# url-kaist/UV-SLAM

Measured on AMD Instinct MI355X. Metric: sliding-window solves/sec (10 KF, 150 pts, 40 lines, 3 VP), higher is better.
Workload: dtype f64; 1 GPU; W10-P150-L40-V3 x 256 independent windows per GPU (BASELINE configs[2]); single window (configs[1]) in single_window, the 20k-point window (configs[3]) in large_window (both with --full); windows_per_gpu=256, frames=11, points=150, lines=40, vp_tagged_lines=30, prior=True, parallelism=replicas x1

## Files before the change

uv-slam_amd/csrc/uvs_solve_kernel.h:

```cpp
#pragma once
#include <hip/hip_runtime.h>
#include <initializer_list>
#include <utility>
#include "../../include/uvs_solver.h"
#include "uvs_layout.h"
#include "uvs_factors.h"

namespace uvsdev {

#ifndef UVS_UNIT
#define UVS_UNIT unit
#endif

#ifndef UVS_X_PLAIN_TID
static __device__ __forceinline__ int lane_tid() { int t = threadIdx.x; asm volatile("" : "+v"(t)); return t; }
#else
static __device__ __forceinline__ int lane_tid() { return threadIdx.x; }
#endif
static constexpr int NT = UVS_NT;
static constexpr int NW = NT / 64;
static constexpr bool ROLES = NT > 256;
static constexpr int ET = ROLES ? 256 : NT;
static constexpr int EW = ET / 64;
static constexpr int GT0 = NT - UVS_GT;
// ... 219 lines not shown
            for (int k = 0; k < 9; ++k) x0[k] = x0g[k];
        }
        const double* xb = (kind == UVS_BLOCK_POSE) ? x + 7 * frame : (kind == UVS_BLOCK_SPEEDBIAS) ? x + 77 + 9 * frame : (kind == UVS_BLOCK_TD) ? x + 183 : x + 176;
        double* dx = c.sh + L_PDX + idx;
        if (size != 7) { for (int k = 0; k < size; ++k) dx[k] = xb[k] - x0[k]; }
        else {
            dx[0] = xb[0] - x0[0]; dx[1] = xb[1] - x0[1]; dx[2] = xb[2] - x0[2];
            double qi[4], e[4]; quat_inv(x0 + 3, qi); quat_mul(qi, xb + 3, e);
            const double sg = (e[3] >= 0.0) ? 2.0 : -2.0;
            dx[3] = sg * e[0]; dx[4] = sg * e[1]; dx[5] = sg * e[2];
        }
    }
}
UVS_DEV double prior_quad(const Ctx& c, int dst = L_PR) {
    DevWinK& h = *c.hdr;
    const int n = h.prior_n, tid = lane_tid();
    double cost = 0.0;
    if (n <= 0) return cost;
    const double* H0 = c.ws + h.w_prior_h0;
    const int parts = (NT / n) < 4 ? (NT / n) : 4;
    const int part = tid / n, row = tid - part * n;
    const double g0v = tid < n ? c.ws[h.w_prior_h0 + UVS_PH_G0(n) + tid] : 0.0, c0v = tid == 0 ? c.ws[h.w_prior_h0 + UVS_PH_C0(n)] : 0.0;
    if (part < parts) {
        const int kb = (n * part) / parts, ke = (n * (part + 1)) / parts;
        double p8[8] = {0, 0, 0, 0, 0, 0, 0, 0};
        for (int k = kb; k < ke; k += PR_UN) {
            double jv[PR_UN];
#pragma unroll
            for (int u = 0; u < PR_UN; ++u) jv[u] = H0[(k + u < ke ? k + u : kb) * n + row];
#pragma unroll
            for (int u = 0; u < PR_UN; ++u) if (k + u < ke) p8[u & 7] += jv[u] * c.sh[L_PDX + k + u];
        }
        c.sh[L_S + 128 * part + row] = ((p8[0] + p8[1]) + (p8[2] + p8[3])) + ((p8[4] + p8[5]) + (p8[6] + p8[7]));
    }
    __syncthreads();
    if (tid < n) {
        double y = c.sh[L_S + tid];
        for (int p = 1; p < parts; ++p) y += c.sh[L_S + 128 * p + tid];
        c.sh[dst + tid] = y;
        cost = c.sh[L_PDX + tid] * (g0v + 0.5 * y);
        if (tid == 0) cost += c0v;
    }
    return cost;
}
UVS_DEV double prior_cost_share(const Ctx& c, int src) {
    DevWinK& h = *c.hdr;
    const int n = h.prior_n, tid = lane_tid();
    double cost = 0.0;
    if (tid < n) {
        cost = c.sh[L_PDX + tid] * (c.ws[h.w_prior_h0 + UVS_PH_G0(n) + tid] + 0.5 * c.sh[src + tid]);
        if (tid == 0) cost += c.ws[h.w_prior_h0 + UVS_PH_C0(n)];
    }
    return cost;
}
UVS_DEV double prior_residual_rows(const Ctx& c) {
    DevWinK& h = *c.hdr;
    const int n = h.prior_n, tid = lane_tid();
    double cost = 0.0;
    if (tid < n) {
        const double* Jr = c.bd + h.d_prior + (size_t)tid * n;
        double s = c.bd[h.d_prior + n * n + tid];
        for (int k = 0; k < n; ++k) s += Jr[k] * c.sh[L_PDX + k];
        c.sh[L_PR + tid] = s;
        cost = 0.5 * s * s;
    }
    return cost;
}

UVS_DEV void cost_imu_raw(const Ctx& c, const double* x, int lane0) {
    DevWinK& h = *c.hdr;
    const int b = lane_tid() - lane0;
    double* rs = c.sh + L_S + 1024;
    if (b >= 0 && b < h.n_imu) {
        const int fi = c.bi[h.i_imu + 2 * b], skip = c.bi[h.i_imu + 2 * b + 1];
        if (!skip) {
            const double* blk = c.bd + h.d_imu + (size_t)b * UVS_IMU_STRIDE;
            double r[15];
            imu_raw(blk, blk + UVS_IMU_JAC, c.o.G, x + 7 * fi, x + 77 + 9 * fi, x + 7 * (fi + 1), x + 77 + 9 * (fi + 1), r, nullptr);
#pragma unroll
            for (int i = 0; i < 15; ++i) rs[16 * b + i] = r[i];
        }
    }
}
template <int PB = CP_PB, int LB = CP_LB>
UVS_DEV double cost_pass(const Ctx& c, const double* x, const double* invd, const double* line, int po0, int po1, int lo0, int lo1, bool with_imu) {
    DevWinK& h = *c.hdr;
    const int tid = lane_tid();
    const double* RF = c.sh + L_RF; const double* ric = c.sh + L_EX; const double* tic = c.sh + L_EX + 9;
    const double* ltrig = line_trig_of(c, line);
    double cost = 0.0;
    long long tq_ = clock64();
#define UVS_CQ(slot) if (c.o.debug == 1 && tid == 0) { const long long t_ = clock64(); c.sh[L_WPROF + slot] += (double)(t_ - tq_); tq_ = t_; }
    const int imu_lane0 = ROLES ? NT - 64 : 0;
#ifndef UVS_X_NO_IMU_WAVE
    if (ROLES && with_imu) cost_imu_raw(c, x, imu_lane0);
#endif
    for (int o0 = po0 + tid; o0 < po1; o0 += PB * NT) {
        int lm[PB], fi[PB], fj[PB]; bool in[PB];
        double pi[PB][3], pj[PB][3], vij[PB][4], idp[PB];
#pragma unroll
        for (int u = 0; u < PB; ++u) {
            const int o = o0 + u * NT; in[u] = o < po1;
            const int oo = in[u] ? o : o0;
            lm[u] = c.bi[h.i_pt_lm + oo]; fi[u] = c.bi[h.i_pt_fi + oo]; fj[u] = c.bi[h.i_pt_fj + oo];
            load_point_obs(c, oo, x[183], pi[u], pj[u], vij[u]);
        }
#pragma unroll
        for (int u = 0; u < PB; ++u) idp[u] = invd[lm[u]];
#pragma unroll
        for (int u = 0; u < PB; ++u) {
            if (!in[u]) continue;
            double r[2];
            point_eval<false, false>(x + 7 * fi[u], RF + 9 * fi[u], pose_of(x, fj[u]), RF + 9 * fj[u], ric, tic, idp[u], pi[u], pj[u], c.o.sqrt_info, r, nullptr, nullptr, nullptr, nullptr);
            double sc; cost += 0.5 * cauchy(c.o.loss_pt, r[0] * r[0] + r[1] * r[1], &sc);
        }
    }
    for (int o0 = lo0 + UVS_COST_LINE_LANE; o0 < lo1; o0 += LB * NT) {
        int lm[LB], fj[LB], hv[LB]; bool in[LB];
        double ms[LB][9], lp[LB][4] = {}, tg[LB][8];
        const int st = h.ln_stride;
#pragma unroll
        for (int u = 0; u < LB; ++u) {
            const int o = o0 + u * NT; in[u] = o < lo1;
            const int oo = in[u] ? o : o0;
            lm[u] = c.bi[h.i_ln_lm + oo]; fj[u] = c.bi[h.i_ln_fj + oo]; hv[u] = c.bi[h.i_ln_vp + oo];
            const double* m = c.bd + h.d_lnmeas + oo;
#pragma unroll
            for (int q = 0; q < 9; ++q) ms[u][q] = m[q * st];
        }
#pragma unroll
        for (int u = 0; u < LB; ++u) {
            if (ltrig) {
#pragma unroll
                for (int q = 0; q < 8; ++q) tg[u][q] = ltrig[8 * lm[u] + q];
            } else {
#pragma unroll
                for (int q = 0; q < 4; ++q) lp[u][q] = line[4 * lm[u] + q];
            }
        }
#pragma unroll
        for (int u = 0; u < LB; ++u) {
            if (!in[u]) continue;
            const double sp[3] = {ms[u][0], ms[u][1], ms[u][2]}, ep[3] = {ms[u][3], ms[u][4], ms[u][5]}, vp[3] = {ms[u][6], ms[u][7], ms[u][8]};
            LineGeom g;
            line_geom<false>(x + 7 * fj[u], x + 7 * fj[u] + 3, RF + 9 * fj[u], ric, tic, lp[u], g, ltrig ? tg[u] : nullptr);
            double r[2], sc;
            line_residual<false>(g, sp, ep, c.o.line_factor, r, nullptr, nullptr);
            cost += 0.5 * cauchy(c.o.loss_ln, r[0] * r[0] + r[1] * r[1], &sc);
            if (hv[u]) { double rv; vp_residual<false>(g, vp, c.o.vp_factor, &rv, nullptr, nullptr); cost += 0.5 * cauchy(c.o.loss_vp, rv * rv, &sc); }
        }
    }
    UVS_CQ(2)
    if (with_imu) {
        double* rs = c.sh + L_S + 1024;
#ifndef UVS_X_NO_IMU_WAVE
        if (!ROLES)
#endif
        cost_imu_raw(c, x, 0);
        __syncthreads();
        const int b = tid >> 4, i = tid & 15;
        if (b < h.n_imu && i < 15 && !c.bi[h.i_imu + 2 * b + 1]) {
            const double* W = c.ws + h.w_imu_w + (size_t)b * UVS_IMU_WS + i * 15;
            double wv[15];
#pragma unroll
            for (int k = 0; k < 15; ++k) wv[k] = (k >= i) ? W[k] : 0.0;
            double sacc = 0.0;
#pragma unroll
            for (int k = 0; k < 15; ++k) sacc += wv[k] * rs[16 * b + k];
            cost += 0.5 * sacc * sacc;
        }
    }
    UVS_CQ(3)
    return cost;
}

typedef double d4_t __attribute__((ext_vector_type(4)));

UVS_DEV double* sblk(double* sh, int i, int j) { return sh + L_S + (((i * (i + 1)) >> 1) + j) * UVS_BLK_SZ; }

UVS_DEV double rcp_newton(double x) {
    double y = __builtin_amdgcn_rcp(x);
    double e = fma(-x, y, 1.0); y = fma(y, e, y);
    e = fma(-x, y, 1.0); y = fma(y, e, y);
    return y;
}

struct MiniCtx { double* sh; struct { int debug; } o; };
template <bool TR = false>
UVS_DEV void chol_update_item(double* sh, int i, int cc, int j0, int j1, int lane, d4_t& acc) {
    const int li = lane & 15, lk = lane >> 4;
    const bool rhs = (i == UVS_NF);
    const double* Bj = sblk(sh, cc, j0) + li * UVS_BLK_LD + lk;
    const double* Ai = rhs ? sh + L_DLT + 16 * j0 + lk : sblk(sh, i, j0) + li * UVS_BLK_LD + lk;
    const int astep = rhs ? 16 : UVS_BLK_SZ;
    if (j0 >= j1) return;
    double a0[4], b0[4], a1[4], b1[4];
#define UVS_CH_LOAD(AV, BV) { _Pragma("unroll") for (int q = 0; q < 4; ++q) { AV[q] = Ai[4 * q]; BV[q] = Bj[4 * q]; } Bj += UVS_BLK_SZ; Ai += astep; }
#define UVS_CH_MFMA(AV, BV) { _Pragma("unroll") for (int q = 0; q < 4; ++q) acc = TR ? __builtin_amdgcn_mfma_f64_16x16x4f64(BV[q], AV[q], acc, 0, 0, 1) : __builtin_amdgcn_mfma_f64_16x16x4f64(AV[q], BV[q], acc, 0, 0, 1); }
    UVS_CH_LOAD(a0, b0)
    for (int j = j0;;) {
        if (j + 1 < j1) UVS_CH_LOAD(a1, b1)
        UVS_CH_MFMA(a0, b0)
        if (++j >= j1) break;
        if (j + 1 < j1) UVS_CH_LOAD(a0, b0)
        UVS_CH_MFMA(a1, b1)
        if (++j >= j1) break;
    }
#undef UVS_CH_LOAD
#undef UVS_CH_MFMA
}
UVS_DEV d4_t chol_load_item(double* sh, int i, int cc, int lane) {
    const int li = lane & 15, lk = lane >> 4;
    d4_t acc;
    if (i == UVS_NF) { const double bv0 = sh[L_DLT + 16 * cc + li]; acc[0] = (lk == 0) ? bv0 : 0.0; acc[1] = 0.0; acc[2] = 0.0; acc[3] = 0.0; }
    else if (i == cc) {
        const double* Dk = sblk(sh, cc, cc);
#pragma unroll
        for (int q = 0; q < 4; ++q) { const int r = lk + 4 * q; const int hi_ = r >= li ? r : li, lo_ = r >= li ? li : r; acc[q] = Dk[hi_ * UVS_BLK_LD + lo_]; }
    } else {
        const double* Cb = sblk(sh, i, cc) + lk * UVS_BLK_LD + li;
#pragma unroll
        for (int q = 0; q < 4; ++q) acc[q] = Cb[4 * q * UVS_BLK_LD];
    }
    return acc;
}
UVS_DEV d4_t chol_load_item_t(double* sh, int i, int cc, int lane) {
    const int li = lane & 15, lk = lane >> 4;
    d4_t acc;
    if (i != UVS_NF) {
        const double* Ai = sblk(sh, i, cc) + li * UVS_BLK_LD + lk;
#pragma unroll
        for (int q = 0; q < 4; ++q) acc[q] = Ai[4 * q];
    } else {
#pragma unroll
        for (int q = 0; q < 4; ++q) { const double yv = sh[L_DLT + 16 * cc + 4 * q + lk]; acc[q] = (li == 0) ? yv : 0.0; }
    }
    return acc;
}
UVS_DEV void chol_store_item(double* sh, int i, int cc, int lane, const d4_t& acc) {
    const int li = lane & 15, lk = lane >> 4;
    if (i == UVS_NF) { if (lk == 0) sh[L_DLT + 16 * cc + li] = acc[0]; }
    else if (i == cc) {
// ... 637 lines not shown
#pragma unroll
                for (int r = 0; r < GR; ++r) { o.p0[r] = pa[r]; o.p1[r] = pa[p1off + r]; }
#pragma unroll
                for (int k = 0; k < 3; ++k) { o.q0[k] = lds2(pb + 2 * k); o.q1[k] = lds2(pb + 6 + 2 * k); }
                o.rc = lds2(S0 + lo + ((w[0] & UVS_PT_ENTRY_A) ? UVS_PT_RC2 - UVS_PT_A : rcoff));
            },
            [&](int, Ops& o) {
#pragma unroll
                for (int r = 0; r < GR; ++r) {
                    if (dirv) { row_fma(A.v + 6 * r, o.p0[r], o.q0); row_fma(A.v + 6 * r, o.p1[r], o.q1); }
                    if (tdcol) A.v[6 * r] += o.p0[r] * o.q0[0].x + o.p1[r] * o.q0[0].y;
                    if (diag) { A.g[r] += o.p0[r] * o.rc.x + o.p1[r] * o.rc.y; A.hd[r] += o.p0[r] * o.p0[r] + o.p1[r] * o.p1[r]; }
                }
            });
    }
}

template <bool DELTA = false>
UVS_DEV void gather_lines(int grp, const int* lists, const double* S0, GAcc& A, int goff = 0, int eoff = 0) {
    const int g = (lane_tid() - GT0) / UVS_GLANES, r0 = GR * (lane_tid() % UVS_GLANES);
    const bool on = grp >= 0;
    const bool diag = on && ((grp >> 8) & 1);
    const int* ent = lists + LIST_HDR;
    {
        struct Ops { double ea[4][GR]; d2_t y[4][3]; double gg[DELTA ? GR : 1]; };
        const int e0 = on ? lists[g] : 0, e1 = on ? lists[g + 1] : 0;
        gather_walk<1, Ops>(ent, e0, e1,
            [&](int, const int* w, Ops& o) {
                const int lo = w[0] & 0x7fff;
                const double* pa = S0 + lo + r0;
                const double* pb = S0 + ((unsigned)w[0] >> 16);
#pragma unroll
                for (int q = 0; q < 4; ++q) {
#pragma unroll
                    for (int r = 0; r < GR; ++r) o.ea[q][r] = pa[6 * q + r];
                    o.y[q][0] = lds2(pb + 6 * q); o.y[q][1] = lds2(pb + 6 * q + 2); o.y[q][2] = lds2(pb + 6 * q + 4);
                }
                if (DELTA) {
                    const double* pg = S0 + goff + 6 * ((lo - eoff) / UVS_LN_EY) + r0;
#pragma unroll
                    for (int r = 0; r < GR; ++r) o.gg[r] = pg[r];
                }
            },
            [&](int, Ops& o) {
#pragma unroll
                for (int q = 0; q < 4; ++q)
#pragma unroll
                    for (int r = 0; r < GR; ++r) row_fma(A.v + 6 * r, -o.ea[q][r], o.y[q]);
                if (DELTA) {
#pragma unroll
                    for (int r = 0; r < GR; ++r) A.g[r] -= diag ? o.gg[r] : 0.0;
                }
            });
    }
    if (DELTA) return;
    {
        struct Ops { double p[3][GR]; d2_t q[3][3], rc01; double rc2; };
        const int e0 = on ? lists[UVS_NGRP + 1 + g] : 0, e1 = on ? lists[UVS_NGRP + 2 + g] : 0;
        gather_walk<1, Ops>(ent, e0, e1,
            [&](int, const int* w, Ops& o) {
                const double* R = S0 + w[0];
#pragma unroll
                for (int k = 0; k < 3; ++k) {
#pragma unroll
                    for (int r = 0; r < GR; ++r) o.p[k][r] = R[UVS_LN_JP + 6 * k + r0 + r];
                    o.q[k][0] = lds2(R + UVS_LN_JP + 6 * k); o.q[k][1] = lds2(R + UVS_LN_JP + 6 * k + 2); o.q[k][2] = lds2(R + UVS_LN_JP + 6 * k + 4);
                }
                o.rc01 = lds2(R); o.rc2 = R[UVS_LN_RV];
            },
            [&](int, Ops& o) {
#pragma unroll
                for (int r = 0; r < GR; ++r) {
#pragma unroll
                    for (int k = 0; k < 3; ++k) { row_fma(A.v + 6 * r, o.p[k][r], o.q[k]); A.hd[r] += o.p[k][r] * o.p[k][r]; }
                    A.g[r] += o.p[0][r] * o.rc01.x + o.p[1][r] * o.rc01.y + o.p[2][r] * o.rc2;
                }
            });
    }
}

static constexpr int IMU_JLD = 48;
static constexpr int IMU_WOFF = 16 * IMU_JLD;
static constexpr int IMU_BLK = IMU_WOFF + UVS_BLK_SZ;
#ifndef UVS_IMU_SLOT_SWAP
#define UVS_IMU_SLOT_SWAP 1
#endif
static constexpr int IMU_SLOTS = (UVS_NF - 1 + NW - 1) / NW;
UVS_DEV int imu_block_of(int wv, int s) {
    if (NW == 8 && UVS_IMU_SLOT_SWAP) return s == 0 ? wv : (wv == 0 ? 9 : wv == 1 ? 8 : UVS_NF);
    return wv + s * NW;
}
struct ImuN { d4_t n00[IMU_SLOTS], n10[IMU_SLOTS], n11[IMU_SLOTS]; int fi[IMU_SLOTS]; bool act[IMU_SLOTS]; };

UVS_DEV double lin_prep(const Ctx& c, const double* x, int mode = 0) {
    UVS_PROF(c, P_MISC);
    const int tid = lane_tid(), n = c.hdr->prior_n;
    if (mode == 0) {
        stage_rotations(c, x);
        prior_dx(c, x);
        __syncthreads();
        return prior_quad(c);
    }
    if (mode == 2) { stage_rotations(c, x); prior_dx(c, x); __syncthreads(); }
    else if (tid < n) c.sh[L_PR + tid] = c.sh[L_PRC + tid];
    __syncthreads();
    return prior_cost_share(c, L_PR);
}
UVS_DEV void lin_imu_stage(const Ctx& c, const double* x) {
    DevWinK& h = *c.hdr;
    double* sh = c.sh;
    const int tid = lane_tid(), lane = tid & 63, wv = tid >> 6;
    __syncthreads();
    UVS_PROF(c, P_GATHER);
    double* IM = sh + L_S;
    constexpr int WPL = ((UVS_NF - 1) * 225 + ET - 1) / ET;
    double wreg[WPL];
#pragma unroll
    for (int q = 0; q < WPL; ++q) {
        const int t = tid + q * ET, tc = t < h.n_imu * 225 ? t : 0, b = tc / 225, e = tc - 225 * b;
        wreg[q] = c.ws[h.w_imu_w + (size_t)b * UVS_IMU_WS + e];
    }
    for (int t = tid; t < h.n_imu * IMU_BLK; t += ET) IM[t] = 0.0;
    UVS_TLOG(c, 40);
    __syncthreads();
    UVS_TLOG(c, 41);
    if (lane < h.n_imu && wv < 4 && !c.bi[h.i_imu + 2 * lane + 1]) {
        const int fi = c.bi[h.i_imu + 2 * lane];
        const double* blk = c.bd + h.d_imu + (size_t)lane * UVS_IMU_STRIDE;
        double* T = IM + IMU_BLK * lane;
        const double* pi_ = x + 7 * fi; const double* si_ = x + 77 + 9 * fi; const double* pj_ = x + 7 * (fi + 1); const double* sj_ = x + 77 + 9 * (fi + 1);
        double r[15];
        if (EW < 4) { imu_raw<IMU_JLD, 1, false>(blk, blk + UVS_IMU_JAC, c.o.G, pi_, si_, pj_, sj_, r, T); for (int i = 0; i < 15; ++i) T[i * IMU_JLD + 31] = r[i]; }
        else if (wv == 0) { imu_raw<IMU_JLD, 1, false, 1>(blk, blk + UVS_IMU_JAC, c.o.G, pi_, si_, pj_, sj_, r, T); for (int i = 0; i < 15; ++i) T[i * IMU_JLD + 31] = r[i]; }
        else if (wv == 1) imu_raw<IMU_JLD, 1, false, 2>(blk, blk + UVS_IMU_JAC, c.o.G, pi_, si_, pj_, sj_, r, T);
        else if (wv == 2) imu_raw<IMU_JLD, 1, false, 4>(blk, blk + UVS_IMU_JAC, c.o.G, pi_, si_, pj_, sj_, r, T);
        else imu_raw<IMU_JLD, 1, false, 8>(blk, blk + UVS_IMU_JAC, c.o.G, pi_, si_, pj_, sj_, r, T);
    }
#pragma unroll
    for (int q = 0; q < WPL; ++q) {
        const int t = tid + q * ET;
        if (t < h.n_imu * 225) { const int b = t / 225, e = t - 225 * b, i = e / 15, k = e - 15 * i; IM[IMU_BLK * b + IMU_WOFF + i * UVS_BLK_LD + k] = wreg[q]; }
    }
    UVS_TLOG(c, 42);
    __syncthreads();
    UVS_TLOG(c, 43);
}
UVS_DEV double lin_imu_tiles(const Ctx& c, ImuN& N) {
    DevWinK& h = *c.hdr;
    double* sh = c.sh;
    const int tid = lane_tid(), lane = tid & 63, wv = UVS_KWAVE(tid), li = lane & 15, lk = lane >> 4;
    double cost = 0.0;
    double* IM = sh + L_S;
    IntK* itab = (IntK*)c.bi + h.i_imu;
    bool act[IMU_SLOTS];
#pragma unroll
    for (int s = 0; s < IMU_SLOTS; ++s) {
        const int b = imu_block_of(wv, s);
        act[s] = b < h.n_imu && !itab[2 * (b < h.n_imu ? b : 0) + 1];
        N.act[s] = act[s]; N.fi[s] = itab[2 * (b < h.n_imu ? b : 0)];
        if (act[s]) {
            double* Jb = IM + IMU_BLK * b; const double* Wb = Jb + IMU_WOFF;
            d4_t t0 = {0.0, 0.0, 0.0, 0.0}, t1 = t0;
            double wa[4], j0[4], j1[4];
#pragma unroll
            for (int q = 0; q < 4; ++q) { wa[q] = Wb[li * UVS_BLK_LD + 4 * q + lk]; j0[q] = Jb[(4 * q + lk) * IMU_JLD + li]; j1[q] = Jb[(4 * q + lk) * IMU_JLD + 16 + li]; }
#pragma unroll
            for (int q = 0; q < 4; ++q) { t0 = __builtin_amdgcn_mfma_f64_16x16x4f64(wa[q], j0[q], t0, 0, 0, 0); t1 = __builtin_amdgcn_mfma_f64_16x16x4f64(wa[q], j1[q], t1, 0, 0, 0); }
#pragma unroll
            for (int q = 0; q < 4; ++q) { Jb[(lk + 4 * q) * IMU_JLD + li] = t0[q]; Jb[(lk + 4 * q) * IMU_JLD + 16 + li] = t1[q]; }
        }
    }
    wave_sync();
#pragma unroll
    for (int s = 0; s < IMU_SLOTS; ++s) {
        const int b = imu_block_of(wv, s);
        d4_t n00 = {0.0, 0.0, 0.0, 0.0}, n10 = n00, n11 = n00;
        if (act[s]) {
            const double* Jb = IM + IMU_BLK * b;
            double j0[4], j1[4];
#pragma unroll
            for (int q = 0; q < 4; ++q) { j0[q] = Jb[(4 * q + lk) * IMU_JLD + li]; j1[q] = Jb[(4 * q + lk) * IMU_JLD + 16 + li]; }
#pragma unroll
            for (int q = 0; q < 4; ++q) {
                n00 = __builtin_amdgcn_mfma_f64_16x16x4f64(j0[q], j0[q], n00, 0, 0, 0);
                n10 = __builtin_amdgcn_mfma_f64_16x16x4f64(j1[q], j0[q], n10, 0, 0, 0);
                n11 = __builtin_amdgcn_mfma_f64_16x16x4f64(j1[q], j1[q], n11, 0, 0, 0);
            }
            if (lane == 63) cost += 0.5 * n11[3];
        }
        N.n00[s] = n00; N.n10[s] = n10; N.n11[s] = n11;
    }
    UVS_PROF(c, P_AS_IMU);
    return cost;
}
UVS_DEV double lin_imu(const Ctx& c, const double* x, ImuN& N) { lin_imu_stage(c, x); return lin_imu_tiles(c, N); }
UVS_DEV double lin_frames(const Ctx& c, const double* x, ImuN& N) { const double pc = lin_prep(c, x); return pc + lin_imu(c, x, N); }

UVS_DEV void spd4_inverse(const double* H, const double* gl, double* X, double* hg) {
    double L[10];
    double i0, i1, i2, i3;
    rsqrt_pair(H[0], &L[0], &i0);
    L[1] = H[1] * i0; rsqrt_pair(H[2] - L[1] * L[1], &L[2], &i1);
    L[3] = H[3] * i0; L[4] = (H[4] - L[3] * L[1]) * i1; rsqrt_pair(H[5] - L[3] * L[3] - L[4] * L[4], &L[5], &i2);
    L[6] = H[6] * i0; L[7] = (H[7] - L[6] * L[1]) * i1; L[8] = (H[8] - L[6] * L[3] - L[7] * L[4]) * i2;
    rsqrt_pair(H[9] - L[6] * L[6] - L[7] * L[7] - L[8] * L[8], &L[9], &i3);
// ... 873 lines not shown
    }
    if (mode != 2) asm_prior(c);
    __syncthreads();
    UVS_PROF(c, P_AS_ADD);
    if (mode == 1) return;
    asm_finish(c, x, first, radius, cost, gmax_lm, mode);
    UVS_PROF(c, P_ASSEMBLE);
}

static constexpr int ROLE_PARTS_OFF = (UVS_NF - 1) * IMU_BLK;
static_assert(ROLE_PARTS_OFF + (8 * GR + 1) * UVS_GT <= UVS_S_DOUBLES, "IMU staging + part sums exceed the S region");
UVS_DEV void role_barriers(int n) { for (int i = 0; i < n; ++i) __syncthreads(); }
UVS_DEV void gacc_store(const Ctx& c, const GAcc& A) {
    double* W = c.ws + c.hdr->w_gacc + (lane_tid() - GT0);
#pragma unroll
    for (int q = 0; q < 6 * GR; ++q) __builtin_nontemporal_store(A.v[q], W + q * UVS_GT);
#pragma unroll
    for (int q = 0; q < GR; ++q) { __builtin_nontemporal_store(A.g[q], W + (6 * GR + q) * UVS_GT); __builtin_nontemporal_store(A.hd[q], W + (7 * GR + q) * UVS_GT); }
}
UVS_DEV void gacc_load(const Ctx& c, GAcc& A) {
    const double* W = c.ws + c.hdr->w_gacc + (lane_tid() - GT0);
#pragma unroll
    for (int q = 0; q < 6 * GR; ++q) A.v[q] = W[q * UVS_GT];
#pragma unroll
    for (int q = 0; q < GR; ++q) { A.g[q] = W[(6 * GR + q) * UVS_GT]; A.hd[q] = W[(7 * GR + q) * UVS_GT]; }
}
UVS_DEV void linearize_roles(const Ctx& c, const double* x, const double* invd, const double* line, bool first, double radius, int prep_mode, bool redamp) {
    DevWinK& h = *c.hdr;
    const bool ev = role_eval();
    { const double pc = lin_prep(c, x, redamp ? 2 : prep_mode); if (!redamp) lacc_set(c.sh, pc, 0.0); }
    double ic = 0.0;
    UVS_TLOG(c, 20);
    PriorAdd pa;
    ImuN N;
    if (ev) {
        ChunkDesc d = chunk_desc(c, 0);
        for (int ch = 0; ch < h.n_chunks; ++ch) {
            if (redamp) redamp_prep(c, d, radius);
            else {
                chunk_eval(c, d, x, invd, line, first, radius);
            }
            if (ch + 1 < h.n_chunks) {
                d = chunk_desc(c, ch + 1);
#ifdef UVS_CHUNK_TOUCH
                if (!redamp) chunk_touch(c, d, invd, line);
#endif
            }
        }
        UVS_TLOG(c, 21);
        lin_imu_stage(c, x);
#ifndef UVS_X_NO_PRIOR_AHEAD
        asm_prior_load(c, pa);
#endif
        ic = lin_imu_tiles(c, N);
        UVS_TLOG(c, 22);
        __syncthreads();
        asm_zero(c);
        __syncthreads();
        UVS_TLOG(c, 23);
        __syncthreads();
        UVS_TLOG(c, 24);
        asm_imu(c, N);
        UVS_TLOG(c, 25);
    } else {
        const int grp = gather_group(c);
        GAcc A;
        if (redamp) gacc_load(c, A); else gacc_zero(A);
        ChunkDesc d = chunk_desc(c, 0);
        for (int ch = 0; ch < h.n_chunks; ++ch) {
            if (redamp) { role_barriers(redamp_barriers(d)); redamp_gather(c, d, grp, A); }
            else {
                __syncthreads();
                if (LISTS_BY_GATHERERS) copy_lists_gatherers(c, d);
                AnchorPre ap; ap.b0 = 0; ap.b1 = 0; ap.sc = 1.0;
                if (ANCHOR_BY_GATHERERS && d.type == 0) pt_anchor_pre(c, d, first, ap);
                __syncthreads();
                if (ANCHOR_BY_GATHERERS && d.type == 0) pt_anchor_pass(c, d, first, radius, ap);
                role_barriers(chunk_eval_barriers(d) - 2);
                chunk_gather(c, d, grp, A);
            }
            if (ch + 1 < h.n_chunks) d = chunk_desc(c, ch + 1);
        }
        __syncthreads();
        if (h.redamp_ok && c.o.redamp) gacc_store(c, A);
        GAcc& T = A;
        gacc_gather_parts(T, grp, c.sh + L_S + ROLE_PARTS_OFF);
#ifndef UVS_X_NO_PRIOR_AHEAD
        asm_prior_load(c, pa);
#endif
        ic = lin_imu_tiles(c, N);
        __syncthreads();
        asm_zero(c);
        __syncthreads();
        asm_part0(c, grp, T);
        __syncthreads();
        asm_imu(c, N);
    }
#ifndef UVS_X_NO_PRIOR_AHEAD
    asm_prior_add(c, pa);
#else
    asm_prior(c);
#endif
    __syncthreads();
    UVS_TLOG(c, 26);
    asm_finish(c, x, first && !redamp, radius, lacc_cost(c.sh) + ic, lacc_gmax(c.sh), 0);
    UVS_TLOG(c, 27);
}

UVS_DEV void linearize(const Ctx& c, const double* x, const double* invd, const double* line, bool first, double radius, int prep_mode, GAcc& A) {
    if (ROLES) { linearize_roles(c, x, invd, line, first, radius, prep_mode, false); return; }
    DevWinK& h = *c.hdr;
    const int grp = gather_group(c);
    gacc_zero(A);
    { const double pc = lin_prep(c, x, prep_mode); lacc_set(c.sh, pc, 0.0); }
    {
        ChunkDesc d = chunk_desc(c, 0);
        for (int ch = 0; ch < h.n_chunks; ++ch) {
            chunk_eval(c, d, x, invd, line, first, radius);
            chunk_gather(c, d, grp, A);
            if (ch + 1 < h.n_chunks) d = chunk_desc(c, ch + 1);
        }
    }
    ImuN N;
    const double ic = lin_imu(c, x, N);
    lin_assemble(c, x, first, radius, grp, A, N, lacc_cost(c.sh) + ic, lacc_gmax(c.sh));
}

UVS_DEV void relinearize_damping(const Ctx& c, const double* x, double radius, GAcc& A) {
    if (ROLES) { linearize_roles(c, x, nullptr, nullptr, false, radius, 2, true); return; }
    DevWinK& h = *c.hdr;
    const int grp = gather_group(c);
    (void)lin_prep(c, x, 2);
    {
        ChunkDesc d = chunk_desc(c, 0);
        for (int ch = 0; ch < h.n_chunks; ++ch) {
            redamp_prep(c, d, radius);
            redamp_gather(c, d, grp, A);
            if (ch + 1 < h.n_chunks) d = chunk_desc(c, ch + 1);
        }
    }
    ImuN N;
    const double ic = lin_imu(c, x, N);
    lin_assemble(c, x, false, radius, grp, A, N, lacc_cost(c.sh) + ic, lacc_gmax(c.sh));
}

#ifndef UVS_BS_FRAME_LANE0
#define UVS_BS_FRAME_LANE0 192
#endif
template <int LNBT = BS_LNB, int PSB = 4, bool STREAM = false>
UVS_DEV void backsub_candidate(const Ctx& c, const double* invd, const double* line, double* invd_c, double* line_c,
                                  int pk0, int pk1, int lk0, int lk1, bool with_frames, double* sums_out, double* lstep = nullptr) {
    DevWinK& h = *c.hdr;
    double* sh = c.sh;
    const int tid = lane_tid();
    const double* d = sh + L_DLT;
    double gd = 0.0, dd2 = 0.0, step2 = 0.0, xc2 = 0.0;
    const bool td_on = UVS_KPIN(h.td_on) != 0;
    const bool ex_on = UVS_KPIN(h.ex_on) != 0, relo_on = h.relo_on != 0;
    double* ltrig_c = const_cast<double*>(line_trig_of(c, line_c));
    const bool relo2 = h.relo2 != 0;
    const int i_pt_fi = UVS_KPIN(h.i_pt_fi), i_pt_fj = UVS_KPIN(h.i_pt_fj), i_ln_fj = UVS_KPIN(h.i_ln_fj), pt_xslots = UVS_KPIN(h.pt_xslots);
    if (relo2) relo2_backsub(c);
    else if (relo_on) {
        if (tid < 6) sh[L_DLT + 16 * UVS_RELO_FRAME + tid] = d[UVS_EX_INDEX(tid)];
        __syncthreads();
    }
    if (with_frames && tid < UVS_RD && ((tid & 15) < 15 || (td_on && tid == UVS_TD_INDEX) || ((ex_on | relo_on) && tid < 96))) { gd += sh[L_G + tid] * d[tid]; dd2 += sh[L_DD + tid] * d[tid] * d[tid]; }
// ... 356 lines not shown
    const long long t_wall0 = wall_clock64();
    while (true) {
        if (it >= o.max_it && !first) { term = UVS_TERM_NO_CONVERGENCE; break; }
        if (o.max_ticks > 0 && !first) {
            __syncthreads();
            if (tid == 0) sh[L_CTRL + C_TIMEUP] = (wall_clock64() - t_wall0 >= o.max_ticks) ? 1.0 : 0.0;
            __syncthreads();
            if (sh[L_CTRL + C_TIMEUP] != 0.0) { term = UVS_TERM_MAX_TIME; break; }
        }
        if (need_lin) {
#ifndef UVS_X_NO_REDAMP
            if (prep_mode == 2 && !first && h.redamp_ok && o.redamp) relinearize_damping(c, sh + L_X, radius, gacc);
            else
#endif
            linearize(c, sh + L_X, invd[cur], line[cur], first, radius, prep_mode, gacc);
            need_lin = false;
            const double lc = sh[L_CTRL + C_COST];
            gmax = sh[L_CTRL + C_GMAX];
            if (first) {
                const double xn2 = ambient_sqnorm(c, sh + L_X, invd[0], line[0]);
                x_norm = sqrt(xn2); cost = lc; first = false;
                if (tid == 0) { rep->initial_cost = cost; rep->cost[0] = cost; rep->radius[0] = radius; rep->gradient_max_norm[0] = gmax; rep->accepted[0] = 1; }
                if (!isfinite(cost)) { term = UVS_TERM_NUMERIC_FAILURE; status = UVS_ERR_NUMERIC; break; }
            } else if (pending > 0) {
                cost = lc;
                if (tid == 0) { rep->cost[pending] = cost; rep->gradient_max_norm[pending] = gmax; }
            }
            pending = 0;
        }
        if (it >= o.max_it) { term = UVS_TERM_NO_CONVERGENCE; break; }
        if (gmax <= o.gtol) { term = UVS_TERM_GRADIENT_TOL; break; }
        if (radius <= o.rmin) { term = UVS_TERM_MIN_RADIUS; break; }
        ++it;
        const int ti = it < UVS_MAX_ITER ? it : UVS_MAX_ITER;
        if (tid < UVS_RD) sh[L_DLT + tid] = -sh[L_G + tid];
        if (o.debug && it == 1 && dbg.S) {
            __syncthreads();
            for (int t = tid; t < UVS_RD * UVS_RD; t += NT) { const int i = t / UVS_RD, j = t - i * UVS_RD; dbg.S[t] = (j <= i) ? sh[L_S + sidx(i, j)] : 0.0; }
            if (tid < UVS_RD) { dbg.g[tid] = sh[L_G + tid]; dbg.hd[tid] = sh[L_HD + tid]; dbg.dd[tid] = sh[L_DD + tid]; }
        }
        UVS_PROF(c, P_MISC);
        UVS_TLOG(c, 30);
        chol_factor(c);
        UVS_PROF(c, P_CHOL);
        UVS_TLOG(c, 31);
        chol_solve(c);
        UVS_PROF(c, P_TRSV);
        UVS_TLOG(c, 32);
        bool ok = sh[L_CTRL + C_CHOLOK] != 0.0;
        backsub_candidate(c, invd[cur], line[cur], invd[cur ^ 1], line[cur ^ 1], 0, h.n_points, 0, h.n_lines, true, nullptr,
                          DSTEP ? ds.steps + (size_t)(it - 1) * ds.stride + UVS_DSTEP_FR : nullptr);
        UVS_PROF(c, P_BACKSUB);
        UVS_TLOG(c, 33);
        const double mcc = sh[L_CTRL + C_MCC], step2 = sh[L_CTRL + C_STEP2], xc2 = sh[L_CTRL + C_XC2];
        if (DSTEP) {
            if (tid < UVS_DSTEP_FR) ds.steps[(size_t)(it - 1) * ds.stride + tid] = sh[L_DLT + tid];
            if (tid == 0) { double* sc = ds.scal + (size_t)(it - 1) * UVS_DEBUG_SCAL_LEN; sc[0] = cost; sc[1] = gmax; sc[2] = ok ? 1.0 : 0.0; sc[3] = mcc; sc[4] = step2; }
            if (it >= ds.n) break;
            radius = ds.radii[it]; need_lin = true; prep_mode = 2;
            __syncthreads();
            continue;
        }
        if (o.debug && it == 1 && dbg.S) {
            if (tid < UVS_RD) dbg.step[tid] = sh[L_DLT + tid];
            if (tid == 0) { dbg.scal[0] = cost; dbg.scal[1] = gmax; dbg.scal[2] = ok ? 1.0 : 0.0; dbg.scal[3] = mcc; dbg.scal[4] = step2; }
        }
        if (!isfinite(mcc) || !isfinite(step2)) ok = false;
        if (tid == 0) rep->model_cost_change[ti] = mcc;
        if (!ok || !(mcc > 0.0)) {
            ++invalid;
            radius = radius / decr; decr *= 2.0; need_lin = true; prep_mode = 2;
            if (tid == 0) { rep->accepted[ti] = -1; rep->cost[ti] = cost; rep->candidate_cost[ti] = cost; rep->radius[ti] = radius; rep->gradient_max_norm[ti] = gmax; }
            if (invalid >= o.max_invalid) { term = UVS_TERM_INVALID_STEPS; break; }
            continue;
        }
        invalid = 0;
        __syncthreads();
        long long tc_ = clock64();
        stage_rotations(c, sh + L_XC);
        prior_dx(c, sh + L_XC);
        __syncthreads();
        if (o.debug == 1 && tid == 0) { const long long t_ = clock64(); sh[L_WPROF + 0] += (double)(t_ - tc_); tc_ = t_; }
        UVS_TLOG(c, 34);
        double cc_ = prior_quad(c, L_PRC);
        UVS_TLOG(c, 35);
        if (o.debug == 1 && tid == 0) { const long long t_ = clock64(); sh[L_WPROF + 1] += (double)(t_ - tc_); tc_ = t_; }
        cc_ += cost_pass(c, sh + L_XC, invd[cur ^ 1], line[cur ^ 1], 0, h.n_pt_obs, 0, h.n_ln_obs, true);
        UVS_TLOG(c, 36);
        double s4[4] = {cc_, 0, 0, 0}, mx = 0.0;
        block_reduce(sh, s4, &mx);
        UVS_TLOG(c, 37);
        UVS_PROF(c, P_COST);
        double cand = s4[0];
        if (!isfinite(cand)) cand = 1.7976931348623157e308;
        const double step_norm = sqrt(step2);
        const double rel = (cost - cand) / mcc;
        const bool successful = rel > o.min_rel;
        if (tid == 0) { rep->candidate_cost[ti] = cand; rep->step_norm[ti] = step_norm; rep->relative_decrease[ti] = rel; rep->cost[ti] = cost; rep->radius[ti] = radius; rep->gradient_max_norm[ti] = gmax; }
        bool stop = false;
        if (step_norm <= o.ptol * (x_norm + o.ptol)) { term = UVS_TERM_PARAMETER_TOL; stop = true; }
        else if (fabs(cost - cand) <= o.ftol * cost) { term = UVS_TERM_FUNCTION_TOL; stop = true; }
        if (stop && !(o.keep_cand && successful)) break;
        if (successful) {
            __syncthreads();
            if (tid < UVS_XDIM) sh[L_X + tid] = sh[L_XC + tid];
            cur ^= 1; ++nsucc;
            x_norm = sqrt(xc2);
            { const double t3 = 2.0 * rel - 1.0; radius = radius / fmax(1.0 / 3.0, 1.0 - t3 * t3 * t3); }
            radius = fmin(o.rmax, radius);
            decr = 2.0;
            cost = cand;
            need_lin = true; pending = ti; prep_mode = 1;
            if (tid == 0) { rep->accepted[ti] = 1; rep->cost[ti] = cost; rep->radius[ti] = radius; }
            if (stop) break;
        } else {
            radius = radius / decr; decr *= 2.0; need_lin = true; prep_mode = 2;
            if (tid == 0) { rep->accepted[ti] = 0; rep->radius[ti] = radius; }
        }
    }
    __syncthreads();
    UVS_PROF(c, P_MISC);
    if (o.debug && dbg.scal && tid < P_LAST) dbg.scal[8 + tid] = sh[L_PROF + tid];
    if (o.debug && dbg.scal && tid < 8) dbg.scal[24 + tid] = sh[L_WPROF + tid];
    if (tid < UVS_XDIM) c.ws[h.w_out + tid] = sh[L_X + tid];
    for (int k = tid; k < h.n_points; k += NT) c.ws[h.w_out + UVS_XDIM + k] = invd[cur][k];
    for (int k = tid; k < 4 * h.n_lines; k += NT) c.ws[h.w_out + UVS_XDIM + h.n_points + k] = line[cur][k];
    if (h.out_host) {
        double* od = (double*)h.out_host;
        if (tid < UVS_XDIM) od[tid] = sh[L_X + tid];
        for (int k = tid; k < h.n_points; k += NT) od[UVS_XDIM + k] = invd[cur][k];
        for (int k = tid; k < 4 * h.n_lines; k += NT) od[UVS_XDIM + h.n_points + k] = line[cur][k];
    }
    if (tid == 0) {
        rep->status = status; rep->termination = term; rep->num_iterations = it; rep->num_successful = nsucc; rep->final_cost = cost;
        ((DevWin*)blob)->cur_sel = cur;
    }
}
#ifdef UVS_EMIT_K_SOLVE
__global__ __launch_bounds__(NT) void k_solve(char* blobs, const long long* blob_off, double* ws_all, const long long* ws_off,
                                              KOpts o, uvs_report* reports, DebugOut dbg) {
    extern __shared__ __attribute__((aligned(16))) double sh[];
    k_solve_body<false>(blobs, blob_off, ws_all, ws_off, o, reports, dbg, DebugStep{}, sh);
}
#endif
#ifdef UVS_EMIT_K_SOLVE_DSTEP
__global__ __launch_bounds__(NT) void k_solve_dstep(char* blobs, const long long* blob_off, double* ws_all, const long long* ws_off,
                                                    KOpts o, uvs_report* reports, DebugStep ds) {
    extern __shared__ __attribute__((aligned(16))) double sh[];
    DebugOut dbg; dbg.S = nullptr; dbg.g = nullptr; dbg.hd = nullptr; dbg.dd = nullptr; dbg.step = nullptr; dbg.scal = nullptr;
    k_solve_body<true>(blobs, blob_off, ws_all, ws_off, o, reports, dbg, ds, sh);
}
#endif

static int unit_init(const unsigned char* fa, const unsigned char* fb, int n, std::initializer_list<const void*> kernels) {
    if (n != UVS_NBLK) return UVS_ERR_INVALID_ARG;
    if (hipMemcpyToSymbol(HIP_SYMBOL(c_blk_fa), fa, n) != hipSuccess || hipMemcpyToSymbol(HIP_SYMBOL(c_blk_fb), fb, n) != hipSuccess) return UVS_ERR_HIP;
    for (const void* fn : kernels) if (hipFuncSetAttribute(fn, hipFuncAttributeMaxDynamicSharedMemorySize, (int)LDS_BYTES) != hipSuccess) return UVS_ERR_HIP;
    return UVS_OK;
}
}
```

Before: 192,300 solves/s.

## Fold prior cost into per-thread partials and widen IMU tile zeroing

New measurement: 192,700 solves/s, median of 3. Within noise of the previous version (+0.2%).

```diff
diff --git a/uv-slam_amd/csrc/uvs_solve_kernel.h b/uv-slam_amd/csrc/uvs_solve_kernel.h
--- a/uv-slam_amd/csrc/uvs_solve_kernel.h
+++ b/uv-slam_amd/csrc/uvs_solve_kernel.h
@@ -325,13 +325,42 @@
         }
     }
 }
-template <int PB = CP_PB, int LB = CP_LB>
-UVS_DEV double cost_pass(const Ctx& c, const double* x, const double* invd, const double* line, int po0, int po1, int lo0, int lo1, bool with_imu) {
+#ifdef UVS_X_PRIOR_IN_COST
+static constexpr bool PQ_IN_COST = ROLES;
+#else
+static constexpr bool PQ_IN_COST = false;
+#endif
+static constexpr int PQ_LANE0 = 256, PQ_LANES = 192;
+static_assert(128 * 3 + UVS_MAX_PRIOR_DIM <= 1024, "prior partials meet the IMU residual scratch of cost_pass");
+UVS_DEV void prior_quad_partials(const Ctx& c) {
+    DevWinK& h = *c.hdr;
+    const int n = h.prior_n, l = lane_tid() - PQ_LANE0;
+    if (n <= 0 || l < 0 || l >= PQ_LANES) return;
+    const double* H0 = c.ws + h.w_prior_h0;
+    const int parts = (NT / n) < 4 ? (NT / n) : 4;
+    for (int p = l; p < n * parts; p += PQ_LANES) {
+        const int part = p / n, row = p - part * n;
+        const int kb = (n * part) / parts, ke = (n * (part + 1)) / parts;
+        double p8[8] = {0, 0, 0, 0, 0, 0, 0, 0};
+        for (int k = kb; k < ke; k += PR_UN) {
+            double jv[PR_UN];
+#pragma unroll
+            for (int u = 0; u < PR_UN; ++u) jv[u] = H0[(k + u < ke ? k + u : kb) * n + row];
+#pragma unroll
+            for (int u = 0; u < PR_UN; ++u) if (k + u < ke) p8[u & 7] += jv[u] * c.sh[L_PDX + k + u];
+        }
+        c.sh[L_S + 128 * part + row] = ((p8[0] + p8[1]) + (p8[2] + p8[3])) + ((p8[4] + p8[5]) + (p8[6] + p8[7]));
+    }
+}
+template <int PB = CP_PB, int LB = CP_LB, bool PQ = false>
+UVS_DEV double cost_pass(const Ctx& c, const double* x, const double* invd, const double* line, int po0, int po1, int lo0, int lo1, bool with_imu,
+                         int pq_dst = 0, double* pq_cost = nullptr) {
     DevWinK& h = *c.hdr;
     const int tid = lane_tid();
     const double* RF = c.sh + L_RF; const double* ric = c.sh + L_EX; const double* tic = c.sh + L_EX + 9;
     const double* ltrig = line_trig_of(c, line);
     double cost = 0.0;
+    if (PQ) prior_quad_partials(c);
     long long tq_ = clock64();
 #define UVS_CQ(slot) if (c.o.debug == 1 && tid == 0) { const long long t_ = clock64(); c.sh[L_WPROF + slot] += (double)(t_ - tq_); tq_ = t_; }
     const int imu_lane0 = ROLES ? NT - 64 : 0;
@@ -400,7 +429,19 @@
         if (!ROLES)
 #endif
         cost_imu_raw(c, x, 0);
+        const int pn = PQ ? h.prior_n : 0;
+        double g0v = 0.0, c0v = 0.0;
+        if (PQ && tid < pn) { g0v = c.ws[h.w_prior_h0 + UVS_PH_G0(pn) + tid]; if (tid == 0) c0v = c.ws[h.w_prior_h0 + UVS_PH_C0(pn)]; }
         __syncthreads();
+        if (PQ && tid < pn) {
+            const int parts = (NT / pn) < 4 ? (NT / pn) : 4;
+            double y = c.sh[L_S + tid];
+            for (int p = 1; p < parts; ++p) y += c.sh[L_S + 128 * p + tid];
+            c.sh[pq_dst + tid] = y;
+            double pc = c.sh[L_PDX + tid] * (g0v + 0.5 * y);
+            if (tid == 0) pc += c0v;
+            *pq_cost = pc;
+        }
         const int b = tid >> 4, i = tid & 15;
         if (b < h.n_imu && i < 15 && !c.bi[h.i_imu + 2 * b + 1]) {
             const double* W = c.ws + h.w_imu_w + (size_t)b * UVS_IMU_WS + i * 15;
@@ -1204,6 +1245,7 @@
 static constexpr int IMU_JLD = 48;
 static constexpr int IMU_WOFF = 16 * IMU_JLD;
 static constexpr int IMU_BLK = IMU_WOFF + UVS_BLK_SZ;
+static_assert(IMU_BLK % 2 == 0 && L_S % 2 == 0, "lin_imu_stage zeroes the tiles in sixteen-byte stores");
 #ifndef UVS_IMU_SLOT_SWAP
 #define UVS_IMU_SLOT_SWAP 1
 #endif
@@ -1223,10 +1265,24 @@
         __syncthreads();
         return prior_quad(c);
     }
+#ifndef UVS_X_NO_PREP_AHEAD
+    double g0v = 0.0, c0v = 0.0;
+    if (tid < n) { g0v = c.ws[c.hdr->w_prior_h0 + UVS_PH_G0(n) + tid]; if (tid == 0) c0v = c.ws[c.hdr->w_prior_h0 + UVS_PH_C0(n)]; }
+#endif
     if (mode == 2) { stage_rotations(c, x); prior_dx(c, x); __syncthreads(); }
     else if (tid < n) c.sh[L_PR + tid] = c.sh[L_PRC + tid];
     __syncthreads();
+#ifndef UVS_X_NO_PREP_AHEAD
+    double cost = 0.0;
+    if (tid < n) {
+        cost = c.sh[L_PDX + tid] * (g0v + 0.5 * c.sh[L_PR + tid]);
+        asm volatile("" : "+v"(cost));
+        if (tid == 0) cost += c0v;
+    }
+    return cost;
+#else
     return prior_cost_share(c, L_PR);
+#endif
 }
 UVS_DEV void lin_imu_stage(const Ctx& c, const double* x) {
     DevWinK& h = *c.hdr;
@@ -1242,7 +1298,12 @@
         const int t = tid + q * ET, tc = t < h.n_imu * 225 ? t : 0, b = tc / 225, e = tc - 225 * b;
         wreg[q] = c.ws[h.w_imu_w + (size_t)b * UVS_IMU_WS + e];
     }
+    UVS_TLOG(c, 44);
+#ifndef UVS_X_NO_IMU_ZERO_B128
+    { const d2_t z2 = {0.0, 0.0}; for (int t = tid; t < h.n_imu * (IMU_BLK / 2); t += ET) *(d2_t*)(IM + 2 * t) = z2; }
+#else
     for (int t = tid; t < h.n_imu * IMU_BLK; t += ET) IM[t] = 0.0;
+#endif
     UVS_TLOG(c, 40);
     __syncthreads();
     UVS_TLOG(c, 41);
@@ -2282,7 +2343,9 @@
             if (ch + 1 < h.n_chunks) d = chunk_desc(c, ch + 1);
         }
         __syncthreads();
+        UVS_TLOG(c, 45);
         if (h.redamp_ok && c.o.redamp) gacc_store(c, A);
+        UVS_TLOG(c, 46);
         GAcc& T = A;
         gacc_gather_parts(T, grp, c.sh + L_S + ROLE_PARTS_OFF);
 #ifndef UVS_X_NO_PRIOR_AHEAD
@@ -2805,10 +2868,11 @@
         __syncthreads();
         if (o.debug == 1 && tid == 0) { const long long t_ = clock64(); sh[L_WPROF + 0] += (double)(t_ - tc_); tc_ = t_; }
         UVS_TLOG(c, 34);
-        double cc_ = prior_quad(c, L_PRC);
+        double cc_ = PQ_IN_COST ? 0.0 : prior_quad(c, L_PRC);
         UVS_TLOG(c, 35);
         if (o.debug == 1 && tid == 0) { const long long t_ = clock64(); sh[L_WPROF + 1] += (double)(t_ - tc_); tc_ = t_; }
-        cc_ += cost_pass(c, sh + L_XC, invd[cur ^ 1], line[cur ^ 1], 0, h.n_pt_obs, 0, h.n_ln_obs, true);
+        if (PQ_IN_COST) { const double cp_ = cost_pass<CP_PB, CP_LB, true>(c, sh + L_XC, invd[cur ^ 1], line[cur ^ 1], 0, h.n_pt_obs, 0, h.n_ln_obs, true, L_PRC, &cc_); cc_ += cp_; }
+        else cc_ += cost_pass(c, sh + L_XC, invd[cur ^ 1], line[cur ^ 1], 0, h.n_pt_obs, 0, h.n_ln_obs, true);
         UVS_TLOG(c, 36);
         double s4[4] = {cc_, 0, 0, 0}, mx = 0.0;
         block_reduce(sh, s4, &mx);
```
